# silence-tang/GaussianIP

Measured on AMD Instinct MI355X. Metric: raster_fwd_bwd_mpix_per_s, higher is better.
Workload: dtype f32; 1 GPU; BASELINE.json configs[1]: 100000 Gaussians (synthetic human surface, SMPL-X-style init), 1024x1024, 4 views per optimizer step, raster forward+backward; gaussians=100000, height=1024, width=1024, prewarm_steps=0, repeats=11, full=False, sh_degree=0, dist_world_size=1, gpus_visible=1, parallelism=1 GPU

## Files before the change

### gaussianip_amd/csrc/render_forward.hip

```cpp
#include <stdlib.h>

#include "gip_internal.h"

#ifndef FWD_PAIRS
#define FWD_PAIRS 4
#endif
#define FWD_THREADS 512
typedef float v2f __attribute__((ext_vector_type(2)));
typedef float v4f __attribute__((ext_vector_type(4)));

__device__ __forceinline__ float xchg32(float x, int hh) {
  float a = x, b = x;
  asm volatile("s_nop 1\n\tv_permlane32_swap_b32 %0, %1\n\ts_nop 1" : "+v"(a), "+v"(b));
  return hh ? a : b;
}

__device__ __forceinline__ void both32(float x, float& lo, float& hi) {
  lo = x; hi = x;
  asm volatile("s_nop 1\n\tv_permlane32_swap_b32 %0, %1\n\ts_nop 1" : "+v"(lo), "+v"(hi));
}

__device__ __forceinline__ int ffs_clear(unsigned long long& m) {
  int j;
  asm volatile("s_ff1_i32_b64 %0, %1\n\ts_bitset0_b64 %1, %0" : "=&s"(j), "+s"(m));
  return j;
}

__global__ void __launch_bounds__(FWD_THREADS)
gip_render_forward_kernel(GipKernelParams kp, const uint32_t* __restrict__ tile_order,
                          const uint32_t* __restrict__ tile_start, const unsigned long long* __restrict__ keys,
                          const GipRecord* __restrict__ records, const float* __restrict__ bg,
                          float* __restrict__ out_color, float* __restrict__ out_depth, float* __restrict__ out_alpha,
                          uint32_t* __restrict__ n_contrib, float* __restrict__ final_T, const uint32_t* __restrict__ ckpt_start,
                          float* __restrict__ checkpoints) {
  const uint32_t pos = blockIdx.x;
  const uint32_t vt = tile_order[pos];
  const uint32_t v = vt / kp.T, tile = vt - v * kp.T;
  const uint32_t tx = tile % kp.tiles_x, ty = tile / kp.tiles_x;
  const int lane = threadIdx.x & 63, wave = threadIdx.x >> 6;
  const int hh = lane >> 5, pl = lane & 31;
  const int lx = ((wave & 1) << 3) | (pl & 7), ly = ((wave >> 1) << 2) | (pl >> 3);
  const int px = tx * GIP_TILE + lx, py = ty * GIP_TILE + ly;
  const bool inside = px < kp.W && py < kp.H;
  const v2f pxy = {(float)px, (float)py};
  const float tile_x0 = (float)(tx * GIP_TILE), tile_y0 = (float)(ty * GIP_TILE);
  const int cpix = ((((ly >> 3) << 1) | (lx >> 3)) << 6) | ((ly & 7) << 3) | (lx & 7);

  const uint32_t start = tile_start[vt];
  uint32_t end = tile_start[vt + 1];
  if (end > kp.capacity) end = kp.capacity;
  if (end < start) end = start;
  const GipRecord* recs = records + (size_t)v * kp.P;

  constexpr int FWD_SLOTS = (FWD_THREADS / 64) * 65;
  __shared__ v2f s_xy[FWD_SLOTS];
  __shared__ v4f s_con[FWD_SLOTS];
  __shared__ v4f s_col[FWD_SLOTS];
  __shared__ uint32_t s_mask[FWD_THREADS];
  if (threadIdx.x < FWD_THREADS / 64) {
    s_xy[threadIdx.x * 65] = (v2f){0.f, 0.f};
    s_con[threadIdx.x * 65] = (v4f){0.f, 0.f, 0.f, 0.f};
    s_col[threadIdx.x * 65] = (v4f){0.f, 0.f, 0.f, 0.f};
  }
  const int sidx = threadIdx.x + (threadIdx.x >> 6) + 1;

  bool done = !inside;
  float T = 1.0f, Wt = 0.f;
  v2f CG = {0.f, 0.f}, BD = {0.f, 0.f};
  uint32_t last_contributor = 0;
  int last_off = -1;

  uint32_t g_next = 0xffffffffu, g_next2 = 0xffffffffu;
  float4 r0 = make_float4(0.f, 0.f, 0.f, 0.f), r1 = r0, r2 = r0;
  if (start + threadIdx.x < end) g_next = (uint32_t)keys[start + threadIdx.x];
  if (start + FWD_THREADS + threadIdx.x < end) g_next2 = (uint32_t)keys[start + FWD_THREADS + threadIdx.x];
  if (g_next != 0xffffffffu) {
    const float4* rp = reinterpret_cast<const float4*>(recs + g_next);
    r0 = rp[0]; r1 = rp[1]; r2 = rp[2];
  }

  for (uint32_t base = start; base < end; base += FWD_THREADS) {
    if (__syncthreads_count(done) == FWD_THREADS) break;
    const uint32_t k = base + threadIdx.x;
    if (k < end) {
      const float4 q0 = r0, q1 = r1, q2 = r2;
      s_xy[sidx] = (v2f){q0.x, q0.y};
      s_con[sidx] = (v4f){q1.x * -0.72134752044448170f, q1.z * -0.72134752044448170f, q1.y * -1.4426950408889634f, q0.w};
      s_col[sidx] = (v4f){q2.x, q2.y, q2.z, q0.z};
      uint32_t mask = 0xff;
      const float t2 = 2.0f * __logf(255.0f * q0.w) + 0.02f;
      const float det = q1.x * q1.z - q1.y * q1.y;
      if (t2 <= 0.f) {
        mask = 0;
      } else if (det > 0.f) {
        const float inv = t2 / det;
        const float hx = sqrtf(inv * q1.z) * 1.01f + 0.05f, hy = sqrtf(inv * q1.x) * 1.01f + 0.05f;
        const float rx = q0.x - tile_x0, ry = q0.y - tile_y0;
        const uint32_t cols = (rx - hx <= 7.f ? 1u : 0u) | (rx + hx >= 8.f ? 2u : 0u);
        const float ylo = ry - hy, yhi = ry + hy;
        const float hd = 0.5f * (q1.x - q1.z);
        const float lmax = 0.5f * (q1.x + q1.z) + sqrtf(__builtin_fmaf(hd, hd, q1.y * q1.y));
        const float rad = sqrtf(inv * lmax) * 1.01f + 0.05f;
        const float rad2 = rad * rad;
        const float ex0 = fmaxf(fmaxf(-rx, rx - 7.f), 0.f), ex1 = fmaxf(fmaxf(8.f - rx, rx - 15.f), 0.f);
        const float ex0s = ex0 * ex0, ex1s = ex1 * ex1;
        mask = 0;
#pragma unroll
        for (int band = 0; band < 4; band++) {
          const float ey = fmaxf(fmaxf((float)(4 * band) - ry, ry - (float)(4 * band + 3)), 0.f);
          const float eys = ey * ey;
          const uint32_t near = (ex0s + eys <= rad2 ? 1u : 0u) | (ex1s + eys <= rad2 ? 2u : 0u);
          if (ylo <= (float)(4 * band + 3) && yhi >= (float)(4 * band)) mask |= (cols & near) << (2 * band);
        }
      }
      s_mask[threadIdx.x] = mask;
    }
    g_next = g_next2;
    g_next2 = (k + 2 * FWD_THREADS < end) ? (uint32_t)keys[k + 2 * FWD_THREADS] : 0xffffffffu;
    if (g_next != 0xffffffffu) {
      const float4* rp = reinterpret_cast<const float4*>(recs + g_next);
      r0 = rp[0]; r1 = rp[1]; r2 = rp[2];
    }
    __syncthreads();
    const int cnt = min((uint32_t)FWD_THREADS, end - base);
    if (!__all(done)) {
      for (int c0 = 0; c0 < cnt; c0 += 64) {
        const uint32_t rel = (base - start) + c0;
        if (rel != 0 && (rel % GIP_SEGMENT) == 0) {
          const float s0 = CG.x + xchg32(CG.x, hh), s1 = CG.y + xchg32(CG.y, hh), s2 = BD.x + xchg32(BD.x, hh), sd = BD.y + xchg32(BD.y, hh);
          const uint32_t slot = ckpt_start[vt] + rel / GIP_SEGMENT - 1;
          if (slot < kp.ckpt_capacity && hh == 0 && !kp.forward_only && !done) {
            float* cp = checkpoints + (size_t)slot * (GIP_CKPT_FLOATS * GIP_BLOCK) + cpix;
            cp[0] = T; cp[GIP_BLOCK] = s0; cp[2 * GIP_BLOCK] = s1; cp[3 * GIP_BLOCK] = s2; cp[4 * GIP_BLOCK] = sd;
          }
        }
        const int e = c0 + lane;
        const uint32_t mk = e < cnt ? s_mask[e] : 0u;
        unsigned long long m = __ballot((mk >> wave) & 1u);
        const int cbase16 = ((c0 >> 6) * 65 + 1) << 4;
        bool wave_done = false;
        while (m) {
          int ja[FWD_PAIRS];
          float al[FWD_PAIRS];
          v4f cc[FWD_PAIRS];
#pragma unroll
          for (int u = 0; u < FWD_PAIRS; u++) {
            const int j1 = ffs_clear(m), j2 = ffs_clear(m);
            const int a1 = cbase16 + (j1 << 4), a2 = cbase16 + (j2 << 4);
            ja[u] = hh ? a2 : a1;
            const v2f d = *(const v2f*)((const char*)s_xy + (ja[u] >> 1)) - pxy;
            const v4f co = *(const v4f*)((const char*)s_con + ja[u]);
            cc[u] = *(const v4f*)((const char*)s_col + ja[u]);
            const v2f t = co.xy * d;
            const float power = __builtin_fmaf(d.x, __builtin_fmaf(co.z, d.y, t.x), t.y * d.y);
            const float a = fminf(GIP_ALPHA_MAX, co.w * __builtin_amdgcn_exp2f(power));
            al[u] = (power <= 0.0f && a >= GIP_ALPHA_MIN) ? a : 0.f;
          }
          const unsigned long long done_before = __ballot(done);
#pragma unroll
          for (int u = 0; u < FWD_PAIRS; u++) {
            float a_e, a_o;
            both32(al[u], a_e, a_o);
            a_e = done ? 0.f : a_e;
            const float t1 = __builtin_fmaf(-a_e, T, T);
            const bool stop1 = t1 < GIP_T_MIN;
            const float T1 = stop1 ? T : t1;
            a_o = (done || stop1) ? 0.f : a_o;
            const float t2 = __builtin_fmaf(-a_o, T1, T1);
            const bool stop2 = t2 < GIP_T_MIN;
            const float w_e = stop1 ? 0.f : a_e * T, w_o = stop2 ? 0.f : a_o * T1;
            const float w = hh ? w_o : w_e;
            CG = __builtin_elementwise_fma(cc[u].xy, (v2f){w, w}, CG);
            BD = __builtin_elementwise_fma(cc[u].zw, (v2f){w, w}, BD);
            Wt += w;
            last_off = w > 0.f ? ja[u] : last_off;
            T = stop2 ? T1 : t2;
            done = done || stop1 || stop2;
          }
          if (__ballot(done) != done_before) {
            if (__all(done)) { wave_done = true; break; }
          }
        }
        if (wave_done) break;
      }
    }
    if (last_off >= 0) {
      const uint32_t slot = (uint32_t)last_off >> 4;
      last_contributor = (base - start) + slot - slot / 65u;
      last_off = -1;
    }
  }

  float C0 = CG.x, C1 = CG.y, C2 = BD.x, Dp = BD.y;
  C0 += xchg32(C0, hh); C1 += xchg32(C1, hh); C2 += xchg32(C2, hh); Wt += xchg32(Wt, hh); Dp += xchg32(Dp, hh);
  const uint32_t lc_other = __float_as_uint(xchg32(__uint_as_float(last_contributor), hh));
  last_contributor = max(last_contributor, lc_other);
  if (inside && hh == 0) {
    const size_t HW = (size_t)kp.H * kp.W;
    const size_t pix = (size_t)py * kp.W + px;
    float* oc = out_color + (size_t)v * 3 * HW;
    oc[pix] = C0 + T * bg[0];
    oc[HW + pix] = C1 + T * bg[1];
    oc[2 * HW + pix] = C2 + T * bg[2];
    out_depth[(size_t)v * HW + pix] = Dp;
    out_alpha[(size_t)v * HW + pix] = Wt;
    if (!kp.forward_only) {
      n_contrib[(size_t)v * HW + pix] = last_contributor;
      final_T[(size_t)v * HW + pix] = T;
    }
  }
}


void gip_launch_render_forward(const GipKernelParams& kp, const float* bg, GipStatePtrs st, float* color, float* depth,
                               float* alpha, hipStream_t s) {
  hipLaunchKernelGGL(gip_render_forward_kernel, dim3(kp.V * kp.T), dim3(FWD_THREADS), 0, s, kp, st.tile_order,
                     st.tile_start, st.keys, st.records, bg, color, depth, alpha, st.n_contrib, st.final_T, st.ckpt_start,
                     st.checkpoints);
}
```

Baseline: 8513 Mpix/s.

## Split long forward tiles into two half-tile blocks with 4-way Gaussian interleave

Long tiles (by a length class from the raster header) get two blocks, each covering an 8-row half of the tile. Within a half, four lane groups each take every fourth Gaussian and combine transmittance through permlane16/32 swaps. The aim is to shorten the critical-path tiles that dominate the forward tail by adding parallelism per tile. It costs extra blocks, redundant loading and culling of each Gaussian list, a heavier sequential compositing scan per step, and it depends on header class boundaries and tile_order putting long tiles first.

After: 8351 Mpix/s, median of 2. -1.9%, worse.

```diff
diff --git a/gaussianip_amd/csrc/render_forward.hip b/gaussianip_amd/csrc/render_forward.hip
--- a/gaussianip_amd/csrc/render_forward.hip
+++ b/gaussianip_amd/csrc/render_forward.hip
@@ -20,47 +20,83 @@
   asm volatile("s_nop 1\n\tv_permlane32_swap_b32 %0, %1\n\ts_nop 1" : "+v"(lo), "+v"(hi));
 }
 
+__device__ __forceinline__ void all16(float x, float& r0, float& r1, float& r2, float& r3) {
+  float lo = x, hi = x;
+  asm volatile("s_nop 1\n\tv_permlane32_swap_b32 %0, %1\n\ts_nop 1" : "+v"(lo), "+v"(hi));
+  r0 = lo; r1 = lo; r2 = hi; r3 = hi;
+  asm volatile("s_nop 1\n\tv_permlane16_swap_b32 %0, %1\n\tv_permlane16_swap_b32 %2, %3\n\ts_nop 1"
+               : "+v"(r0), "+v"(r1), "+v"(r2), "+v"(r3));
+}
+
+template <int G>
+__device__ __forceinline__ float group_sum(float x, int grp) {
+  if constexpr (G == 2) {
+    return x + xchg32(x, grp);
+  } else {
+    float r0, r1, r2, r3;
+    all16(x, r0, r1, r2, r3);
+    return (r0 + r1) + (r2 + r3);
+  }
+}
+
 __device__ __forceinline__ int ffs_clear(unsigned long long& m) {
   int j;
   asm volatile("s_ff1_i32_b64 %0, %1\n\ts_bitset0_b64 %1, %0" : "=&s"(j), "+s"(m));
   return j;
 }
 
-__global__ void __launch_bounds__(FWD_THREADS)
-gip_render_forward_kernel(GipKernelParams kp, const uint32_t* __restrict__ tile_order,
-                          const uint32_t* __restrict__ tile_start, const unsigned long long* __restrict__ keys,
-                          const GipRecord* __restrict__ records, const float* __restrict__ bg,
-                          float* __restrict__ out_color, float* __restrict__ out_depth, float* __restrict__ out_alpha,
-                          uint32_t* __restrict__ n_contrib, float* __restrict__ final_T, const uint32_t* __restrict__ ckpt_start,
-                          float* __restrict__ checkpoints) {
-  const uint32_t pos = blockIdx.x;
-  const uint32_t vt = tile_order[pos];
+#ifndef FWD_LONG_MIN
+#define FWD_LONG_MIN 1024
+#endif
+#define FWD_LONG_SLOTS 256
+#ifndef FWD_LONG_PAIRS
+#define FWD_LONG_PAIRS 2
+#endif
+extern "C" { int gip_dbg_fwd_long = -1; }
+
+#ifdef GIP_FWD_TIMELINE
+static unsigned long long* g_fwd_timeline = nullptr;
+extern "C" void gip_dbg_fwd_timeline(void* buf) { g_fwd_timeline = (unsigned long long*)buf; }
+#define FWD_TIMELINE_PARAM , unsigned long long* __restrict__ timeline
+#define FWD_TIMELINE_ARG , g_fwd_timeline
+#else
+#define FWD_TIMELINE_PARAM
+#define FWD_TIMELINE_ARG
+#endif
+
+constexpr int FWD_SLOTS = (FWD_THREADS / 64) * 65;
+struct FwdShared {
+  v2f xy[FWD_SLOTS];
+  v4f con[FWD_SLOTS];
+  v4f col[FWD_SLOTS];
+  uint32_t mask[FWD_THREADS];
+};
+
+template <int G, int U>
+__device__ __forceinline__ void fwd_tile(const GipKernelParams& kp, FwdShared& sh, const uint32_t vt, const uint32_t start,
+                                         const uint32_t end, const int half, const unsigned long long* __restrict__ keys,
+                                         const GipRecord* __restrict__ records, const float* __restrict__ bg,
+                                         float* __restrict__ out_color, float* __restrict__ out_depth, float* __restrict__ out_alpha,
+                                         uint32_t* __restrict__ n_contrib, float* __restrict__ final_T,
+                                         const uint32_t* __restrict__ ckpt_start, float* __restrict__ checkpoints) {
   const uint32_t v = vt / kp.T, tile = vt - v * kp.T;
   const uint32_t tx = tile % kp.tiles_x, ty = tile / kp.tiles_x;
   const int lane = threadIdx.x & 63, wave = threadIdx.x >> 6;
-  const int hh = lane >> 5, pl = lane & 31;
-  const int lx = ((wave & 1) << 3) | (pl & 7), ly = ((wave >> 1) << 2) | (pl >> 3);
+  constexpr int PIX = 64 / G;
+  const int grp = lane / PIX, pl = lane & (PIX - 1);
+  const int lx = G == 2 ? ((wave & 1) << 3) | (pl & 7) : ((wave & 3) << 2) | (pl & 3);
+  const int ly = G == 2 ? ((wave >> 1) << 2) | (pl >> 3) : (half << 3) | ((wave >> 2) << 2) | (pl >> 2);
   const int px = tx * GIP_TILE + lx, py = ty * GIP_TILE + ly;
   const bool inside = px < kp.W && py < kp.H;
   const v2f pxy = {(float)px, (float)py};
-  const float tile_x0 = (float)(tx * GIP_TILE), tile_y0 = (float)(ty * GIP_TILE);
+  const float tile_x0 = (float)(tx * GIP_TILE), tile_y0 = (float)(ty * GIP_TILE + (G == 2 ? 0 : half << 3));
   const int cpix = ((((ly >> 3) << 1) | (lx >> 3)) << 6) | ((ly & 7) << 3) | (lx & 7);
-
-  const uint32_t start = tile_start[vt];
-  uint32_t end = tile_start[vt + 1];
-  if (end > kp.capacity) end = kp.capacity;
-  if (end < start) end = start;
   const GipRecord* recs = records + (size_t)v * kp.P;
 
-  constexpr int FWD_SLOTS = (FWD_THREADS / 64) * 65;
-  __shared__ v2f s_xy[FWD_SLOTS];
-  __shared__ v4f s_con[FWD_SLOTS];
-  __shared__ v4f s_col[FWD_SLOTS];
-  __shared__ uint32_t s_mask[FWD_THREADS];
   if (threadIdx.x < FWD_THREADS / 64) {
-    s_xy[threadIdx.x * 65] = (v2f){0.f, 0.f};
-    s_con[threadIdx.x * 65] = (v4f){0.f, 0.f, 0.f, 0.f};
-    s_col[threadIdx.x * 65] = (v4f){0.f, 0.f, 0.f, 0.f};
+    sh.xy[threadIdx.x * 65] = (v2f){0.f, 0.f};
+    sh.con[threadIdx.x * 65] = (v4f){0.f, 0.f, 0.f, 0.f};
+    sh.col[threadIdx.x * 65] = (v4f){0.f, 0.f, 0.f, 0.f};
   }
   const int sidx = threadIdx.x + (threadIdx.x >> 6) + 1;
 
@@ -84,9 +120,9 @@
     const uint32_t k = base + threadIdx.x;
     if (k < end) {
       const float4 q0 = r0, q1 = r1, q2 = r2;
-      s_xy[sidx] = (v2f){q0.x, q0.y};
-      s_con[sidx] = (v4f){q1.x * -0.72134752044448170f, q1.z * -0.72134752044448170f, q1.y * -1.4426950408889634f, q0.w};
-      s_col[sidx] = (v4f){q2.x, q2.y, q2.z, q0.z};
+      sh.xy[sidx] = (v2f){q0.x, q0.y};
+      sh.con[sidx] = (v4f){q1.x * -0.72134752044448170f, q1.z * -0.72134752044448170f, q1.y * -1.4426950408889634f, q0.w};
+      sh.col[sidx] = (v4f){q2.x, q2.y, q2.z, q0.z};
       uint32_t mask = 0xff;
       const float t2 = 2.0f * __logf(255.0f * q0.w) + 0.02f;
       const float det = q1.x * q1.z - q1.y * q1.y;
@@ -96,24 +132,45 @@
         const float inv = t2 / det;
         const float hx = sqrtf(inv * q1.z) * 1.01f + 0.05f, hy = sqrtf(inv * q1.x) * 1.01f + 0.05f;
         const float rx = q0.x - tile_x0, ry = q0.y - tile_y0;
-        const uint32_t cols = (rx - hx <= 7.f ? 1u : 0u) | (rx + hx >= 8.f ? 2u : 0u);
         const float ylo = ry - hy, yhi = ry + hy;
         const float hd = 0.5f * (q1.x - q1.z);
         const float lmax = 0.5f * (q1.x + q1.z) + sqrtf(__builtin_fmaf(hd, hd, q1.y * q1.y));
         const float rad = sqrtf(inv * lmax) * 1.01f + 0.05f;
         const float rad2 = rad * rad;
-        const float ex0 = fmaxf(fmaxf(-rx, rx - 7.f), 0.f), ex1 = fmaxf(fmaxf(8.f - rx, rx - 15.f), 0.f);
-        const float ex0s = ex0 * ex0, ex1s = ex1 * ex1;
         mask = 0;
-#pragma unroll
-        for (int band = 0; band < 4; band++) {
-          const float ey = fmaxf(fmaxf((float)(4 * band) - ry, ry - (float)(4 * band + 3)), 0.f);
-          const float eys = ey * ey;
-          const uint32_t near = (ex0s + eys <= rad2 ? 1u : 0u) | (ex1s + eys <= rad2 ? 2u : 0u);
-          if (ylo <= (float)(4 * band + 3) && yhi >= (float)(4 * band)) mask |= (cols & near) << (2 * band);
+        if constexpr (G == 2) {
+          const uint32_t cols = (rx - hx <= 7.f ? 1u : 0u) | (rx + hx >= 8.f ? 2u : 0u);
+          const float ex0 = fmaxf(fmaxf(-rx, rx - 7.f), 0.f), ex1 = fmaxf(fmaxf(8.f - rx, rx - 15.f), 0.f);
+          const float ex0s = ex0 * ex0, ex1s = ex1 * ex1;
+#pragma unroll
+          for (int band = 0; band < 4; band++) {
+            const float ey = fmaxf(fmaxf((float)(4 * band) - ry, ry - (float)(4 * band + 3)), 0.f);
+            const float eys = ey * ey;
+            const uint32_t near = (ex0s + eys <= rad2 ? 1u : 0u) | (ex1s + eys <= rad2 ? 2u : 0u);
+            if (ylo <= (float)(4 * band + 3) && yhi >= (float)(4 * band)) mask |= (cols & near) << (2 * band);
+          }
+        } else {
+          const float xlo = rx - hx, xhi = rx + hx;
+          uint32_t cols = 0;
+          float exs[4];
+#pragma unroll
+          for (int col = 0; col < 4; col++) {
+            const float ex = fmaxf(fmaxf((float)(4 * col) - rx, rx - (float)(4 * col + 3)), 0.f);
+            exs[col] = ex * ex;
+            cols |= (xlo <= (float)(4 * col + 3) && xhi >= (float)(4 * col)) ? 1u << col : 0u;
+          }
+#pragma unroll
+          for (int band = 0; band < 2; band++) {
+            const float ey = fmaxf(fmaxf((float)(4 * band) - ry, ry - (float)(4 * band + 3)), 0.f);
+            const float eys = ey * ey;
+            uint32_t near = 0;
+#pragma unroll
+            for (int col = 0; col < 4; col++) near |= (exs[col] + eys <= rad2) ? 1u << col : 0u;
+            if (ylo <= (float)(4 * band + 3) && yhi >= (float)(4 * band)) mask |= (cols & near) << (4 * band);
+          }
         }
       }
-      s_mask[threadIdx.x] = mask;
+      sh.mask[threadIdx.x] = mask;
     }
     g_next = g_next2;
     g_next2 = (k + 2 * FWD_THREADS < end) ? (uint32_t)keys[k + 2 * FWD_THREADS] : 0xffffffffu;
@@ -127,30 +184,37 @@
       for (int c0 = 0; c0 < cnt; c0 += 64) {
         const uint32_t rel = (base - start) + c0;
         if (rel != 0 && (rel % GIP_SEGMENT) == 0) {
-          const float s0 = CG.x + xchg32(CG.x, hh), s1 = CG.y + xchg32(CG.y, hh), s2 = BD.x + xchg32(BD.x, hh), sd = BD.y + xchg32(BD.y, hh);
+          const float s0 = group_sum<G>(CG.x, grp), s1 = group_sum<G>(CG.y, grp), s2 = group_sum<G>(BD.x, grp), sd = group_sum<G>(BD.y, grp);
           const uint32_t slot = ckpt_start[vt] + rel / GIP_SEGMENT - 1;
-          if (slot < kp.ckpt_capacity && hh == 0 && !kp.forward_only && !done) {
+          if (slot < kp.ckpt_capacity && grp == 0 && !kp.forward_only && !done) {
             float* cp = checkpoints + (size_t)slot * (GIP_CKPT_FLOATS * GIP_BLOCK) + cpix;
             cp[0] = T; cp[GIP_BLOCK] = s0; cp[2 * GIP_BLOCK] = s1; cp[3 * GIP_BLOCK] = s2; cp[4 * GIP_BLOCK] = sd;
           }
         }
         const int e = c0 + lane;
-        const uint32_t mk = e < cnt ? s_mask[e] : 0u;
+        const uint32_t mk = e < cnt ? sh.mask[e] : 0u;
         unsigned long long m = __ballot((mk >> wave) & 1u);
         const int cbase16 = ((c0 >> 6) * 65 + 1) << 4;
         bool wave_done = false;
         while (m) {
-          int ja[FWD_PAIRS];
-          float al[FWD_PAIRS];
-          v4f cc[FWD_PAIRS];
-#pragma unroll
-          for (int u = 0; u < FWD_PAIRS; u++) {
+          int ja[U];
+          float al[U];
+          v4f cc[U];
+#pragma unroll
+          for (int u = 0; u < U; u++) {
             const int j1 = ffs_clear(m), j2 = ffs_clear(m);
             const int a1 = cbase16 + (j1 << 4), a2 = cbase16 + (j2 << 4);
-            ja[u] = hh ? a2 : a1;
-            const v2f d = *(const v2f*)((const char*)s_xy + (ja[u] >> 1)) - pxy;
-            const v4f co = *(const v4f*)((const char*)s_con + ja[u]);
-            cc[u] = *(const v4f*)((const char*)s_col + ja[u]);
+            if constexpr (G == 2) {
+              ja[u] = grp ? a2 : a1;
+            } else {
+              const int j3 = ffs_clear(m), j4 = ffs_clear(m);
+              const int a3 = cbase16 + (j3 << 4), a4 = cbase16 + (j4 << 4);
+              const int alo = (grp & 1) ? a2 : a1, ahi = (grp & 1) ? a4 : a3;
+              ja[u] = (grp & 2) ? ahi : alo;
+            }
+            const v2f d = *(const v2f*)((const char*)sh.xy + (ja[u] >> 1)) - pxy;
+            const v4f co = *(const v4f*)((const char*)sh.con + ja[u]);
+            cc[u] = *(const v4f*)((const char*)sh.col + ja[u]);
             const v2f t = co.xy * d;
             const float power = __builtin_fmaf(d.x, __builtin_fmaf(co.z, d.y, t.x), t.y * d.y);
             const float a = fminf(GIP_ALPHA_MAX, co.w * __builtin_amdgcn_exp2f(power));
@@ -158,24 +222,25 @@
           }
           const unsigned long long done_before = __ballot(done);
 #pragma unroll
-          for (int u = 0; u < FWD_PAIRS; u++) {
-            float a_e, a_o;
-            both32(al[u], a_e, a_o);
-            a_e = done ? 0.f : a_e;
-            const float t1 = __builtin_fmaf(-a_e, T, T);
-            const bool stop1 = t1 < GIP_T_MIN;
-            const float T1 = stop1 ? T : t1;
-            a_o = (done || stop1) ? 0.f : a_o;
-            const float t2 = __builtin_fmaf(-a_o, T1, T1);
-            const bool stop2 = t2 < GIP_T_MIN;
-            const float w_e = stop1 ? 0.f : a_e * T, w_o = stop2 ? 0.f : a_o * T1;
-            const float w = hh ? w_o : w_e;
+          for (int u = 0; u < U; u++) {
+            float av[G];
+            if constexpr (G == 2) both32(al[u], av[0], av[1]);
+            else all16(al[u], av[0], av[1], av[2], av[3]);
+            float w = 0.f;
+#pragma unroll
+            for (int g = 0; g < G; g++) {
+              const float a = done ? 0.f : av[g];
+              const float t = __builtin_fmaf(-a, T, T);
+              const bool stop = t < GIP_T_MIN;
+              const float wg = stop ? 0.f : a * T;
+              w = grp == g ? wg : w;
+              T = stop ? T : t;
+              done = done || stop;
+            }
             CG = __builtin_elementwise_fma(cc[u].xy, (v2f){w, w}, CG);
             BD = __builtin_elementwise_fma(cc[u].zw, (v2f){w, w}, BD);
             Wt += w;
             last_off = w > 0.f ? ja[u] : last_off;
-            T = stop2 ? T1 : t2;
-            done = done || stop1 || stop2;
           }
           if (__ballot(done) != done_before) {
             if (__all(done)) { wave_done = true; break; }
@@ -191,11 +256,17 @@
     }
   }
 
-  float C0 = CG.x, C1 = CG.y, C2 = BD.x, Dp = BD.y;
-  C0 += xchg32(C0, hh); C1 += xchg32(C1, hh); C2 += xchg32(C2, hh); Wt += xchg32(Wt, hh); Dp += xchg32(Dp, hh);
-  const uint32_t lc_other = __float_as_uint(xchg32(__uint_as_float(last_contributor), hh));
-  last_contributor = max(last_contributor, lc_other);
-  if (inside && hh == 0) {
+  const float C0 = group_sum<G>(CG.x, grp), C1 = group_sum<G>(CG.y, grp), C2 = group_sum<G>(BD.x, grp), Dp = group_sum<G>(BD.y, grp);
+  Wt = group_sum<G>(Wt, grp);
+  if constexpr (G == 2) {
+    const uint32_t lc_other = __float_as_uint(xchg32(__uint_as_float(last_contributor), grp));
+    last_contributor = max(last_contributor, lc_other);
+  } else {
+    float l0, l1, l2, l3;
+    all16(__uint_as_float(last_contributor), l0, l1, l2, l3);
+    last_contributor = max(max(__float_as_uint(l0), __float_as_uint(l1)), max(__float_as_uint(l2), __float_as_uint(l3)));
+  }
+  if (inside && grp == 0) {
     const size_t HW = (size_t)kp.H * kp.W;
     const size_t pix = (size_t)py * kp.W + px;
     float* oc = out_color + (size_t)v * 3 * HW;
@@ -211,10 +282,54 @@
   }
 }
 
+__global__ void __launch_bounds__(FWD_THREADS)
+gip_render_forward_kernel(GipKernelParams kp, const GipRasterHeader* __restrict__ header, const int long_class, const uint32_t extra,
+                          const uint32_t* __restrict__ tile_order, const uint32_t* __restrict__ tile_start,
+                          const unsigned long long* __restrict__ keys, const GipRecord* __restrict__ records,
+                          const float* __restrict__ bg, float* __restrict__ out_color, float* __restrict__ out_depth,
+                          float* __restrict__ out_alpha, uint32_t* __restrict__ n_contrib, float* __restrict__ final_T,
+                          const uint32_t* __restrict__ ckpt_start, float* __restrict__ checkpoints FWD_TIMELINE_PARAM) {
+#ifdef GIP_FWD_TIMELINE
+  const unsigned long long t_begin = wall_clock64();
+#endif
+  __shared__ FwdShared sh;
+  const uint32_t n_long = extra ? min(header->class_end[long_class], extra) : 0u;
+  uint32_t pos = blockIdx.x;
+  int half = -1;
+  if (pos < extra) {
+    if (pos >= n_long) return;
+    half = 1;
+  } else {
+    pos -= extra;
+    if (pos < n_long) half = 0;
+  }
+  const uint32_t vt = tile_order[pos];
+  const uint32_t start = tile_start[vt];
+  uint32_t end = tile_start[vt + 1];
+  if (end > kp.capacity) end = kp.capacity;
+  if (end < start) end = start;
+  if (half >= 0)
+    fwd_tile<4, FWD_LONG_PAIRS>(kp, sh, vt, start, end, half, keys, records, bg, out_color, out_depth, out_alpha, n_contrib, final_T,
+                                ckpt_start, checkpoints);
+  else
+    fwd_tile<2, FWD_PAIRS>(kp, sh, vt, start, end, 0, keys, records, bg, out_color, out_depth, out_alpha, n_contrib, final_T,
+                           ckpt_start, checkpoints);
+#ifdef GIP_FWD_TIMELINE
+  if (timeline) {
+    unsigned long long* row = timeline + (size_t)blockIdx.x * 16;
+    if (threadIdx.x == 0) { row[0] = t_begin; row[1] = (unsigned long long)(end - start) | ((unsigned long long)(half + 1) << 32); row[2] = vt; }
+    if ((threadIdx.x & 63) == 0) row[3 + (threadIdx.x >> 6)] = wall_clock64();
+  }
+#endif
+}
+
 
 void gip_launch_render_forward(const GipKernelParams& kp, const float* bg, GipStatePtrs st, float* color, float* depth,
                                float* alpha, hipStream_t s) {
-  hipLaunchKernelGGL(gip_render_forward_kernel, dim3(kp.V * kp.T), dim3(FWD_THREADS), 0, s, kp, st.tile_order,
-                     st.tile_start, st.keys, st.records, bg, color, depth, alpha, st.n_contrib, st.final_T, st.ckpt_start,
-                     st.checkpoints);
-}
+  const int min_len = gip_dbg_fwd_long < 0 ? FWD_LONG_MIN : gip_dbg_fwd_long;
+  const int long_class = min_len >= 2048 ? 1 : min_len >= 1024 ? 2 : 0;
+  const uint32_t extra = min_len > 0 ? FWD_LONG_SLOTS : 0;
+  hipLaunchKernelGGL(gip_render_forward_kernel, dim3(extra + kp.V * kp.T), dim3(FWD_THREADS), 0, s, kp, st.header, long_class, extra,
+                     st.tile_order, st.tile_start, st.keys, st.records, bg, color, depth, alpha, st.n_contrib, st.final_T,
+                     st.ckpt_start, st.checkpoints FWD_TIMELINE_ARG);
+}
```
